# kocurvik/mdrp

Measured on NVIDIA B200. Metric: image_pairs_per_sec, higher is better.
Workload: dtype f64

## Files before the change

mdrp_b200/csrc/repose_b200.cu:

```cuda
#include <cuda.h>
#include <cuda_runtime.h>
#include <algorithm>
#include <cstdio>
#include <cstdlib>
#include <cstring>
#include <string>
#include <type_traits>
#include <vector>

#include "rp_kernels.cuh"

using namespace rp;

namespace {

std::string g_create_error;

struct DevBuf {
    void *p = nullptr;
    size_t cap = 0;
    cudaError_t reserve(size_t bytes) {
        if (bytes <= cap) return cudaSuccess;
        if (p) cudaFree(p);
        p = nullptr;
        cap = 0;
        const size_t want = bytes + bytes / 8 + 256;
        cudaError_t e = cudaMalloc(&p, want);
        if (e == cudaSuccess) cap = want;
        return e;
    }
    void release() {
        if (p) cudaFree(p);
        p = nullptr;
        cap = 0;
    }
    template <class T>
    T *as() const { return (T *)p; }
};

enum { B_OFFS, B_PAIRS, B_PTS64, B_PTS32, B_BEAR, B_SAMPLES, B_MODELS, B_HYPITER, B_SCORE, B_COUNT, B_SEGCNT,
       B_ITEMPFX, B_SCALARS, B_EVENTS, B_NEVENTS, B_LOMODELS, B_LOOFEV, B_LOCOUNT, B_PROBLIST, B_LOSCORE,
       B_LOCNT, B_LOITEMPFX, B_BEST, B_FINSTART, B_FINSCORE, B_FINCNT, B_ONES, B_ONEPFX, B_ENABLE, B_STATS,
       B_PTS32P, B_UB, B_LB, B_FIRSTCNT, B_FIRSTPFX, B_B0, B_S0, B_SURVLIST, B_SURVCNT, B_SURVPFX, B_WAVECUR, B_WAVECNT,
       B_MASK, B_IN_X1, B_IN_X2, B_IN_D1, B_IN_D2, B_IN_CAMS, B_TMP0, B_TMP1, B_TMP2,
       B_MASK_B, B_IN_X1_B, B_IN_X2_B, B_IN_D1_B, B_IN_D2_B, B_IN_CAMS_B, B_TMP0_B, B_TMP1_B,
       B_FEAT, B_TCOUT, B_TCLIST, B_TCLISTCNT, B_TCLISTPFX, B_PAIRCNT, B_TCPFX, B_TCSPLIT,
       B_PAIRFLAGS, B_SUB_IDX, B_SUB_SRC, B_SUB_DST, B_SUB_X1, B_SUB_X2, B_SUB_D1, B_SUB_D2, B_SUB_CAMS, B_SUB_MODELS,
       B_SUB_STATS, B_SUB_MASK,
       B_STG_X1, B_STG_X2, B_STG_D1, B_STG_D2, B_STG_X1_B, B_STG_X2_B, B_STG_D1_B, B_STG_D2_B,
       B_QUAL, B_QUAL_B, B_ORDOFFS, B_ORDOFFS_B, B_PERM, B_PERM_B, B_KSORT, B_KSORT_B, B_ORDSCR,
       B_GATHER_Q,
       B_RF_INIT, B_RF_INIT_B, B_RF_SUB, B_RF_SUB_B, B_RF_NINL, B_RF_NINL_B, B_NBUF };

struct Scalars {
    int n_items, n_lo_items, n_one_items, n_prob, n_pairs_scalar, any_flag, reserved0, n_first_items;
    int n_surv_items, bound_work, lm_work, score_work;
    unsigned long long point_scores, lm_iters, n_survivors, evaluated_ps;
    long long n_hyp;
    int n_tc_items, n_tcsel_items;
    unsigned long long tc_evaluated, tc_selected, lm_flops;
};

constexpr int N_EVENTS = 29;

}

struct rp_ctx {
    int device = 0;
    int sms = 148;
    std::string err;
    int64_t launches = 0;
    cudaStream_t stream = nullptr;
    cudaStream_t copy_stream = nullptr;
    DevBuf buf[B_NBUF];
    cudaEvent_t ev[N_EVENTS];
    double last_ms[16] = {0};
    double prev_h2d_ms = 0.0, prev_dev_ms = 0.0;
    int64_t last_cnt[16] = {0};
    size_t workspace_budget = (size_t)80 << 30;
    bool prune = true;
    int head = HB;
    bool waves = true;
    int lm_warp = 0xf;
    int head_small = 32;
    int mid_end = 256;
    int mid_ends[4] = {256, 0, 0, 0}, n_mid = 1;
    bool tc = true;
    int tc_two_pass = -115;
    void *encode_tiled = nullptr;
    int ev_cap0 = EV;
    std::vector<int32_t> pair_status;
    int occ_score[4] = {0}, occ_lm[4] = {0};
};

namespace {

#define CK(call)                                                                                     \
    do {                                                                                             \
        cudaError_t e_ = (call);                                                                     \
        if (e_ != cudaSuccess) {                                                                     \
            char b_[512];                                                                            \
            snprintf(b_, sizeof b_, "%s failed at %s:%d: %s", #call, __FILE__, __LINE__,             \
                     cudaGetErrorString(e_));                                                        \
            ctx->err = b_;                                                                           \
            return RP_ERR_CUDA;                                                                      \
        }                                                                                            \
    } while (0)

#define LAUNCHED()                                                                                   \
    do {                                                                                             \
        ctx->launches++;                                                                             \
        CK(cudaGetLastError());                                                                      \
    } while (0)

inline int cdiv(long long a, long long b) { return (int)((a + b - 1) / b); }

// ... 25 lines not shown
}

template <class K>
int occupancy_grid(rp_ctx *ctx, K kernel, int threads) {
    int nb = 0;
    if (cudaOccupancyMaxActiveBlocksPerMultiprocessor(&nb, kernel, threads, 0) != cudaSuccess || nb < 1) nb = 1;
    return nb * ctx->sms;
}

int launch_score(rp_ctx *ctx, bool pose, bool mask, const ScoreArgs &args, cudaStream_t st) {
    int grid;
    ScoreArgs a = args;
    a.work_counter = &ctx->buf[B_SCALARS].as<Scalars>()->score_work;
    CK(cudaMemsetAsync(a.work_counter, 0, sizeof(int), st));
    if (pose) {
        if (mask) { grid = occupancy_grid(ctx, score_kernel<true, true>, SCORE_THREADS); score_kernel<true, true><<<grid, SCORE_THREADS, 0, st>>>(a); }
        else { grid = occupancy_grid(ctx, score_kernel<true, false>, SCORE_THREADS); score_kernel<true, false><<<grid, SCORE_THREADS, 0, st>>>(a); }
    } else {
        if (mask) { grid = occupancy_grid(ctx, score_kernel<false, true>, SCORE_THREADS); score_kernel<false, true><<<grid, SCORE_THREADS, 0, st>>>(a); }
        else { grid = occupancy_grid(ctx, score_kernel<false, false>, SCORE_THREADS); score_kernel<false, false><<<grid, SCORE_THREADS, 0, st>>>(a); }
    }
    LAUNCHED();
    return RP_OK;
}

int launch_bound(rp_ctx *ctx, bool pose, const BoundArgs &a, cudaStream_t st) {
    CK(cudaMemsetAsync(a.work_counter, 0, sizeof(int), st));
    if (pose) bound_kernel<true><<<occupancy_grid(ctx, bound_kernel<true>, SCORE_THREADS), SCORE_THREADS, 0, st>>>(a);
    else bound_kernel<false><<<occupancy_grid(ctx, bound_kernel<false>, SCORE_THREADS), SCORE_THREADS, 0, st>>>(a);
    LAUNCHED();
    return RP_OK;
}

int launch_lm(rp_ctx *ctx, int variant, const LMArgs &a, long long expected_problems, cudaStream_t st) {
    ctx->launches++;
    (void)expected_problems;
    LMArgs la = a;
    la.work_counter = &ctx->buf[B_SCALARS].as<Scalars>()->lm_work;
    la.warp_kernel = (ctx->lm_warp >> variant) & 1;
    la.warp_single = (ctx->lm_warp >> 4) & 1;
    CK(cudaMemsetAsync(la.work_counter, 0, sizeof(int), st));
    CK((cudaError_t)launch_lm_kernel(ctx->sms, variant, la, st));
    return RP_OK;
}

int launch_solve(rp_ctx *ctx, int variant, const SolveArgs &a, int n_pairs, cudaStream_t st) {
    dim3 grid(a.nseg, n_pairs);
    const bool generic = getenv("RP_SOLVE_GENERIC") != nullptr;
    switch (variant) {
    case RP_CALIB:
        if (generic) solve_kernel<RP_CALIB><<<grid, SOLVE_THREADS, 0, st>>>(a);
        else solve2_kernel<P3PCand><<<grid, SOLVE_THREADS, 0, st>>>(a);
        break;
    case RP_CALIB_SHIFT:
        if (generic) solve_kernel<RP_CALIB_SHIFT><<<grid, SOLVE_THREADS, 0, st>>>(a);
        else solve2_kernel<ShiftCand><<<grid, SOLVE_THREADS, 0, st>>>(a);
        break;
    case RP_SHARED:
        if (generic) solve_kernel<RP_SHARED><<<grid, SOLVE_THREADS, 0, st>>>(a);
        else solve2_kernel<FocalCand><<<grid, SOLVE_THREADS, 0, st>>>(a);
        break;
    default: solve_kernel<RP_VARYING><<<grid, SOLVE_THREADS, 0, st>>>(a); break;
    }
    LAUNCHED();
    return RP_OK;
}

__global__ void valid_ones_kernel(int n_pairs, const PairParams *pairs, int *ones) {
    const int i = blockIdx.x * blockDim.x + threadIdx.x;
    if (i < n_pairs) ones[i] = pairs[i].valid ? 1 : 0;
}

__global__ void stage_points_kernel(int n, const double *x1, const double *x2, double sq_thr, Pt64 *pts64,
// ... 294 lines not shown
            }
        }
        CK(cudaEventRecord(ev[20], st));
        rc = cascade(from, 0, ctx->tc_two_pass, use_tc ? ev[22] : nullptr, ev[21]);
        if (rc) return rc;
    }
    CK(cudaEventRecord(ev[4], st));
    {
        ScanArgs a;
        a.n_pairs = P; a.nseg = nseg; a.seg_count = seg_count; a.score = score; a.count = count;
        a.events = B[B_EVENTS].as<int>(); a.n_events = B[B_NEVENTS].as<int>(); a.ev_cap = ev_cap;
        a.pair_flags = B[B_PAIRFLAGS].as<int>(); a.any_flag = &sc->any_flag;
        scan_kernel<<<cdiv((long long)P * 32, 256), 256, 0, st>>>(a);
        LAUNCHED();
        LoPrepArgs l;
        l.n_pairs = P; l.nseg = nseg; l.events = a.events; l.n_events = a.n_events; l.hyp_iter = hyp_iter; l.ev_cap = ev_cap;
        l.models = models; l.lo_models = B[B_LOMODELS].as<Model>(); l.lo_of_event = B[B_LOOFEV].as<int>();
        l.lo_count = B[B_LOCOUNT].as<int>(); l.prob_list = B[B_PROBLIST].as<int>(); l.n_prob = &sc->n_prob;
        lo_prepare_kernel<<<cdiv(P, 128), 128, 0, st>>>(l);
        LAUNCHED();
    }
    CK(cudaEventRecord(ev[5], st));
    LMArgs la;
    memset(&la, 0, sizeof la);
    la.pairs = pairs; la.pts64 = pts64; la.d1 = io.d1; la.d2 = io.d2;
    la.weight_sampson = opt.weight_sampson; la.gradient_tol = 1e-10; la.step_tol = 1e-8;
    la.initial_lambda = 1e-3; la.min_lambda = 1e-10; la.max_lambda = 1e10;
    la.loss_scale_override = -1.0; la.scale_reproj_override = -1.0;
    la.lm_iters = &sc->lm_iters;
    la.lm_flops = &sc->lm_flops;
    {
        la.prob_list = B[B_PROBLIST].as<int>(); la.n_prob = &sc->n_prob; la.prob_per_pair = ev_cap;
        la.models = B[B_LOMODELS].as<Model>(); la.use_final = 0;
        int rc = launch_lm(ctx, variant, la, (long long)P * 8, st);
        if (rc) return rc;
    }
    CK(cudaEventRecord(ev[6], st));
    {
        build_items_kernel<<<1, 1024, 0, st>>>(P, B[B_LOCOUNT].as<int>(), B[B_LOITEMPFX].as<int>(), &sc->n_lo_items, nullptr);
        LAUNCHED();
        ScoreArgs s2 = sa;
        s2.slot_list = nullptr; s2.list_stride = 0;
        s2.n_groups = P; s2.grp_stride = ev_cap; s2.grp_per_pair = 1; s2.grp_cnt = B[B_LOCOUNT].as<int>();
        s2.item_prefix = B[B_LOITEMPFX].as<int>(); s2.n_items = &sc->n_lo_items; s2.models = B[B_LOMODELS].as<Model>();
        s2.score = B[B_LOSCORE].as<double>(); s2.count = B[B_LOCNT].as<int>(); s2.point_scores = nullptr;
        int rc = launch_score(ctx, pose, false, s2, st);
        if (rc) return rc;
        MergeArgs m;
        m.n_pairs = P; m.nseg = nseg; m.iters = iters; m.pairs = pairs; m.events = B[B_EVENTS].as<int>();
        m.min_iterations = opt.min_iterations; m.max_iterations = opt.max_iterations;
        m.dyn_num_trials_mult = opt.dyn_num_trials_mult; m.log_prob_missing = log(1.0 - opt.success_prob);
        m.hyp_iter = hyp_iter; m.ev_cap = ev_cap; m.pair_flags = B[B_PAIRFLAGS].as<int>(); m.any_flag = &sc->any_flag;
        m.n_events = B[B_NEVENTS].as<int>(); m.lo_of_event = B[B_LOOFEV].as<int>(); m.score = score; m.count = count;
        m.models = models; m.lo_score = B[B_LOSCORE].as<double>(); m.lo_count_inl = B[B_LOCNT].as<int>();
        m.lo_models = B[B_LOMODELS].as<Model>(); m.lo_count = B[B_LOCOUNT].as<int>();
        m.best = B[B_BEST].as<Model>(); m.stats = B[B_STATS].as<rp_stats>(); m.final_start = B[B_FINSTART].as<Model>();
        merge_kernel<<<cdiv(P, 128), 128, 0, st>>>(m);
        LAUNCHED();
        la.prob_list = nullptr; la.n_prob = &sc->n_pairs_scalar; la.prob_per_pair = 1;
        la.models = B[B_FINSTART].as<Model>(); la.use_final = 0;
        rc = launch_lm(ctx, variant, la, P, st);
        if (rc) return rc;
        valid_ones_kernel<<<cdiv(P, 256), 256, 0, st>>>(P, pairs, B[B_ONES].as<int>());
        LAUNCHED();
        build_items_kernel<<<1, 1024, 0, st>>>(P, B[B_ONES].as<int>(), B[B_ONEPFX].as<int>(), &sc->n_one_items, nullptr);
        LAUNCHED();
        ScoreArgs s3 = s2;
        s3.grp_stride = 1; s3.grp_cnt = B[B_ONES].as<int>(); s3.item_prefix = B[B_ONEPFX].as<int>();
        s3.n_items = &sc->n_one_items; s3.models = B[B_FINSTART].as<Model>();
        s3.score = B[B_FINSCORE].as<double>(); s3.count = B[B_FINCNT].as<int>();
        rc = launch_score(ctx, pose, false, s3, st);
        if (rc) return rc;
        Merge2Args m2;
        m2.n_pairs = P; m2.pairs = pairs; m2.refined = B[B_FINSTART].as<Model>(); m2.ref_score = B[B_FINSCORE].as<double>();
        m2.ref_count = B[B_FINCNT].as<int>(); m2.best = B[B_BEST].as<Model>(); m2.stats = B[B_STATS].as<rp_stats>();
        merge2_kernel<<<cdiv(P, 128), 128, 0, st>>>(m2);
        LAUNCHED();
        CK(cudaMemsetAsync(io.masks_out, 0, (size_t)std::max<long long>(N, 1), st));
        ScoreArgs s4 = s3;
        s4.models = B[B_BEST].as<Model>(); s4.mask = io.masks_out;
        rc = launch_score(ctx, pose, true, s4, st);
        if (rc) return rc;
    }
    CK(cudaEventRecord(ev[7], st));
    {
        enable_final_kernel<<<cdiv(P, 256), 256, 0, st>>>(P, B[B_STATS].as<rp_stats>(), B[B_ENABLE].as<int>());
        LAUNCHED();
        la.prob_list = nullptr; la.n_prob = &sc->n_pairs_scalar; la.prob_per_pair = 1;
        la.models = B[B_BEST].as<Model>(); la.use_final = 1; la.mask = io.masks_out; la.enable = B[B_ENABLE].as<int>();
        la.max_iterations = (int)opt.bundle_max_iterations; la.loss_type = opt.loss_type;
        la.gradient_tol = opt.gradient_tol; la.step_tol = opt.step_tol; la.initial_lambda = opt.initial_lambda;
        la.min_lambda = opt.min_lambda; la.max_lambda = opt.max_lambda;
        int rc = launch_lm(ctx, variant, la, P, st);
        if (rc) return rc;
        finalize_kernel<<<cdiv(P, 256), 256, 0, st>>>(P, variant, pairs, B[B_BEST].as<Model>());
        LAUNCHED();
        CK(cudaMemcpyAsync(io.models_out, B[B_BEST].p, sizeof(Model) * P, cudaMemcpyDeviceToDevice, st));
        CK(cudaMemcpyAsync(io.stats_out, B[B_STATS].p, sizeof(rp_stats) * P, cudaMemcpyDeviceToDevice, st));
    }
    CK(cudaEventRecord(ev[8], st));
    CK(cudaMemcpyAsync(&h_sc, sc, sizeof h_sc, cudaMemcpyDeviceToHost, st));
    CK(cudaStreamSynchronize(st));
    for (int i = 0; i < 8; ++i) {
        float ms = 0.f;
        CK(cudaEventElapsedTime(&ms, ev[i], ev[i + 1]));
        ctx->last_ms[i] += ms;
    }
    {
        float ms = 0.f;
        CK(cudaEventElapsedTime(&ms, ev[0], ev[8]));
        ctx->last_ms[8] += ms;
    }
    ctx->last_cnt[0] += h_sc.n_hyp;
    ctx->last_cnt[1] += (int64_t)h_sc.point_scores;
    ctx->last_cnt[2] += h_sc.n_prob + P;
    ctx->last_cnt[3] += (int64_t)h_sc.lm_iters;
    ctx->last_cnt[4] += 1;
    ctx->last_cnt[6] += (int64_t)h_sc.evaluated_ps;
    if (ctx->prune) {
        float msb = 0.f;
        CK(cudaEventElapsedTime(&msb, use_tc ? ev[22] : ev[20], ev[21]));
        ctx->last_ms[11] += msb;
        if (use_tc) {
            CK(cudaEventElapsedTime(&msb, ev[20], ev[22]));
            ctx->last_ms[12] += msb;
        }
    }
    ctx->last_cnt[8] += (int64_t)h_sc.tc_evaluated;
    ctx->last_cnt[9] += (int64_t)h_sc.tc_selected;
    ctx->last_cnt[10] += (int64_t)h_sc.lm_flops;
    ctx->last_cnt[5] += ctx->prune ? (int64_t)h_sc.n_survivors + std::min<int64_t>(h_sc.n_hyp, (int64_t)P * ((ctx->tc && ctx->mid_end > ctx->head_small) ? ctx->head_small : ctx->head)) : h_sc.n_hyp;
    ctx->last_cnt[7] = ctx->head;
    flags.assign((size_t)P, 0);
    if (h_sc.any_flag) {
        CK(cudaMemcpyAsync(flags.data(), B[B_PAIRFLAGS].p, sizeof(int) * (size_t)P, cudaMemcpyDeviceToHost, st));
        CK(cudaStreamSynchronize(st));
    }
    return RP_OK;
}

size_t bytes_per_pair(int iters, long long avg_points, int ev_cap = EV, size_t input_bytes = 0) {
    const int nseg = std::max(1, cdiv(iters, SEG));
    const size_t slots_pp = (size_t)nseg * 4 * SEG;
    return slots_pp * (sizeof(Model) + 4 + 8 + 4 + 12 + 8) + (size_t)iters * 12 + (size_t)ev_cap * (sizeof(Model) + 24) +
           (size_t)avg_points * (sizeof(Pt64) + 32 + sizeof(Bear) + 1 + 128 + input_bytes) + 1024;
}

template <class In>
int launch_widen(rp_ctx *ctx, long long n, const In *x1, const In *x2, const In *d1, const In *d2, double *wx1,
                 double *wx2, double *wd1, double *wd2, cudaStream_t st, const int *perm = nullptr,
                 const long long *offsets = nullptr, long long base = 0, int n_pairs = 0) {
    if (n <= 0) return RP_OK;
    const int grid = std::min<long long>(cdiv(perm ? n : 2 * n, 256), 16LL * ctx->sms);
    widen_inputs_kernel<In><<<grid, 256, 0, st>>>(n, x1, x2, d1, d2, perm, offsets, base, n_pairs, wx1, wx2, wd1, wd2);
    LAUNCHED();
    return RP_OK;
}

int launch_order(rp_ctx *ctx, int P, long long n, const int64_t *h_offsets, const long long *d_offsets, long long base,
                 const float *quality, int *perm, cudaStream_t st) {
    if (n <= 0) return RP_OK;
    long long max_n = 0;
    for (int p = 0; p < P; ++p) max_n = std::max<long long>(max_n, h_offsets[p + 1] - h_offsets[p]);
    OrderArgs a;
    a.offsets = d_offsets; a.base = base; a.quality = quality; a.perm = perm;
    a.smem_cap = (int)std::min<long long>(max_n, ORDER_SMEM_CAP);
    a.gkeys = nullptr; a.gidx = nullptr;
    if (max_n > ORDER_SMEM_CAP) {
        CK(ctx->buf[B_ORDSCR].reserve(12 * (size_t)n));
        a.gkeys = ctx->buf[B_ORDSCR].as<unsigned>();
        a.gidx = (int *)(a.gkeys + 2 * n);
    }
    order_by_quality_kernel<<<P, ORDER_THREADS, (size_t)ORDER_SMEM_PER_POINT * a.smem_cap, st>>>(a);
    LAUNCHED();
    return RP_OK;
}

int launch_scatter_masks(rp_ctx *ctx, int P, long long n, const long long *d_offsets, long long base, const int *perm,
// ... 379 lines not shown
    PairParams *pairs = B[B_PAIRS].as<PairParams>();
    Model *work = B[B_BEST].as<Model>();
    int *enable = B[B_ENABLE].as<int>();
    Scalars h_sc;
    memset(&h_sc, 0, sizeof h_sc);
    h_sc.n_pairs_scalar = P;
    CK(cudaMemcpyAsync(sc, &h_sc, sizeof h_sc, cudaMemcpyHostToDevice, st));
    CK(cudaMemcpyAsync(B[B_OFFS].p, io.h_offsets_rel, sizeof(long long) * (P + 1), cudaMemcpyHostToDevice, st));
    {
        PrepareArgs a;
        a.variant = variant; a.n_pairs = P; a.offsets = B[B_OFFS].as<long long>();
        a.x1 = io.x1; a.x2 = io.x2; a.cams = io.cams;
        a.max_epipolar_error = opt.max_epipolar_error; a.max_reproj_error = opt.max_reproj_error;
        a.loss_scale = opt.loss_scale;
        a.pts64 = B[B_PTS64].as<Pt64>(); a.pts32 = B[B_PTS32].as<float4>(); a.bear = B[B_BEAR].as<Bear>();
        a.pairs = pairs; a.pts32p = B[B_PTS32P].as<float>();
        prepare_kernel<<<cdiv((long long)P * 32, 256), 256, 0, st>>>(a);
        LAUNCHED();
    }
    refine_import_kernel<<<cdiv((long long)P * 32, 256), 256, 0, st>>>(P, variant, pairs, io.subset, io.init, work, enable,
                                                                      io.bstats_out);
    LAUNCHED();
    {
        LMArgs la;
        memset(&la, 0, sizeof la);
        la.pairs = pairs; la.pts64 = B[B_PTS64].as<Pt64>(); la.d1 = io.d1; la.d2 = io.d2;
        la.weight_sampson = opt.weight_sampson;
        la.loss_scale_override = -1.0; la.scale_reproj_override = -1.0;
        la.prob_list = nullptr; la.n_prob = &sc->n_pairs_scalar; la.prob_per_pair = 1;
        la.models = work; la.use_final = 1; la.mask = io.subset; la.enable = enable; la.stats = io.bstats_out;
        la.max_iterations = (int)opt.bundle_max_iterations; la.loss_type = opt.loss_type;
        la.gradient_tol = opt.gradient_tol; la.step_tol = opt.step_tol; la.initial_lambda = opt.initial_lambda;
        la.min_lambda = opt.min_lambda; la.max_lambda = opt.max_lambda;
        int rc = launch_lm(ctx, variant, la, P, st);
        if (rc) return rc;
    }
    if (io.inliers_out) {
        valid_ones_kernel<<<cdiv(P, 256), 256, 0, st>>>(P, pairs, B[B_ONES].as<int>());
        LAUNCHED();
        build_items_kernel<<<1, 1024, 0, st>>>(P, B[B_ONES].as<int>(), B[B_ONEPFX].as<int>(), &sc->n_one_items, nullptr);
        LAUNCHED();
        if (N > 0) CK(cudaMemsetAsync(io.inliers_out, 0, (size_t)N, st));
        ScoreArgs s;
        memset(&s, 0, sizeof s);
        s.n_groups = P; s.grp_stride = 1; s.grp_per_pair = 1; s.grp_cnt = B[B_ONES].as<int>();
        s.item_prefix = B[B_ONEPFX].as<int>(); s.n_items = &sc->n_one_items; s.pairs = pairs; s.models = work;
        s.pts32 = B[B_PTS32].as<float4>(); s.pts64 = B[B_PTS64].as<Pt64>(); s.bear = B[B_BEAR].as<Bear>();
        s.score = B[B_FINSCORE].as<double>(); s.count = B[B_FINCNT].as<int>(); s.mask = io.inliers_out;
        int rc = launch_score(ctx, pose, true, s, st);
        if (rc) return rc;
    }
    refine_export_kernel<<<cdiv(P, 256), 256, 0, st>>>(P, variant, pairs, enable, io.init, work, B[B_FINCNT].as<int>(),
                                                       io.models_out, io.num_inliers_out);
    LAUNCHED();
    return RP_OK;
}

size_t refine_bytes_per_pair(long long avg_points, bool host_io, bool f32) {
    const size_t io_pt = 48 + 1 + 1 + (host_io && f32 ? 24 : 0);
    const size_t io_pair = 2 * sizeof(Model) + sizeof(rp_bundle_stats) + 64 + 8;
    const size_t sets = host_io ? 2 : 1;
    return (size_t)avg_points * (32 + 16 + 16 + 48 + sets * io_pt) + sizeof(PairParams) + sizeof(Model) + 32 +
           sets * io_pair + 64;
}

template <class In>
int refine_impl(rp_ctx *ctx, int variant, int64_t n_pairs, const int64_t *offsets, const In *x1, const In *x2,
                const In *d1, const In *d2, const double *cams, const rp_options *opt_in, const rp_model *init,
                const uint8_t *subset, rp_model *models, rp_bundle_stats *bstats, int64_t *num_inliers, uint8_t *inliers,
                bool host_io, cudaStream_t st) {
    constexpr bool f32 = std::is_same<In, float>::value;
    if (!ctx) return RP_ERR_INVALID;
    if (n_pairs > 0 && (!x1 || !x2 || !d1 || !d2)) return fail(ctx, RP_ERR_INVALID, "null data pointer");
    if (n_pairs > 0 && (!init || !models)) return fail(ctx, RP_ERR_INVALID, "null init / models");
    int rc = check_common(ctx, variant, n_pairs, offsets, opt_in);
    if (rc) return rc;
    CK(cudaSetDevice(ctx->device));
    rp_options opt = *opt_in;
    if (variant == RP_CALIB && opt.estimate_shift) variant = RP_CALIB_SHIFT;
    const bool pose = variant == RP_CALIB || variant == RP_CALIB_SHIFT;
    if (pose && !cams && n_pairs > 0) return fail(ctx, RP_ERR_INVALID, "calibrated variants need cams");
    if (n_pairs == 0) return RP_OK;
    const bool score = num_inliers || inliers;
    const long long Ntot = offsets[n_pairs] - offsets[0];
    int64_t chunk = (int64_t)std::max<size_t>(1, ctx->workspace_budget / refine_bytes_per_pair(Ntot / n_pairs + 1, host_io, f32));
    chunk = std::min<int64_t>(chunk, 32768);
    if (host_io && n_pairs >= 1024) chunk = std::min<int64_t>(chunk, (n_pairs + 3) / 4);
    const int64_t n_chunks = (n_pairs + chunk - 1) / chunk;
    std::vector<int64_t> bounds((size_t)n_chunks + 1);
    for (int64_t i = 0; i <= n_chunks; ++i) bounds[(size_t)i] = (n_pairs * i) / n_chunks;
    DevBuf *B = ctx->buf;
    static const int IN_X1[2] = {B_IN_X1, B_IN_X1_B}, IN_X2[2] = {B_IN_X2, B_IN_X2_B}, IN_D1[2] = {B_IN_D1, B_IN_D1_B},
                     IN_D2[2] = {B_IN_D2, B_IN_D2_B}, IN_CAMS[2] = {B_IN_CAMS, B_IN_CAMS_B}, STG_X1[2] = {B_STG_X1, B_STG_X1_B},
                     STG_X2[2] = {B_STG_X2, B_STG_X2_B}, STG_D1[2] = {B_STG_D1, B_STG_D1_B}, STG_D2[2] = {B_STG_D2, B_STG_D2_B},
                     INIT[2] = {B_RF_INIT, B_RF_INIT_B}, SUB[2] = {B_RF_SUB, B_RF_SUB_B}, OUT_M[2] = {B_TMP0, B_TMP0_B},
                     OUT_S[2] = {B_TMP1, B_TMP1_B}, OUT_K[2] = {B_MASK, B_MASK_B}, OUT_N[2] = {B_RF_NINL, B_RF_NINL_B};
// ... 104 lines not shown

extern "C" {

int rp_create(int device, rp_ctx **out) {
    if (!out) return RP_ERR_INVALID;
    *out = nullptr;
    int ndev = 0;
    cudaError_t e = cudaGetDeviceCount(&ndev);
    if (e != cudaSuccess || ndev == 0) {
        g_create_error = std::string("no CUDA device: ") + cudaGetErrorString(e);
        return RP_ERR_NO_DEVICE;
    }
    if (device < 0 || device >= ndev) {
        g_create_error = "device index out of range";
        return RP_ERR_INVALID;
    }
    cudaDeviceProp prop;
    if (cudaGetDeviceProperties(&prop, device) != cudaSuccess || prop.major < 10) {
        g_create_error = "device is not sm_100-class (this library only ships sm_100a code)";
        return RP_ERR_NO_DEVICE;
    }
    rp_ctx *ctx = new rp_ctx();
    ctx->device = device;
    ctx->sms = prop.multiProcessorCount;
    if (cudaSetDevice(device) != cudaSuccess || cudaStreamCreateWithFlags(&ctx->stream, cudaStreamNonBlocking) != cudaSuccess ||
        cudaStreamCreateWithFlags(&ctx->copy_stream, cudaStreamNonBlocking) != cudaSuccess) {
        g_create_error = "cudaSetDevice / stream creation failed";
        delete ctx;
        return RP_ERR_CUDA;
    }
    for (auto &ev : ctx->ev) cudaEventCreate(&ev);
    if (const char *np = getenv("RP_NO_PRUNE")) ctx->prune = !(np[0] == '1');
    if (const char *nw = getenv("RP_NO_WAVES")) ctx->waves = !(nw[0] == '1');
    if (const char *lw = getenv("RP_LM_WARP")) ctx->lm_warp = atoi(lw) & 0x1f;
    if (const char *hs = getenv("RP_HEAD_SMALL")) { const int v = atoi(hs); if (v >= 0 && v <= 256 && v % 32 == 0) ctx->head_small = v; }
    if (const char *me = getenv("RP_MID_END")) {
        int n = 0, vals[4] = {0, 0, 0, 0};
        bool ok = true;
        for (const char *p = me; *p && n < 4;) {
            const int v = atoi(p);
            if (v < 0 || v > SEG || v % 32 != 0 || (n && v <= vals[n - 1])) ok = false;
            vals[n++] = v;
            while (*p && *p != ',') ++p;
            if (*p == ',') ++p;
        }
        if (ok && n) { ctx->n_mid = n; for (int k = 0; k < 4; ++k) ctx->mid_ends[k] = vals[k]; ctx->mid_end = vals[n - 1]; }
    }
    if (const char *nt = getenv("RP_NO_TC")) ctx->tc = !(nt[0] == '1');
    if (const char *sp = getenv("RP_TC_SPLIT")) { const int v = atoi(sp); if (v >= 1 && v <= 15) ctx->tc_two_pass = v; }
    if (const char *ap = getenv("RP_TC_ADAPT_PCT")) { const int v = atoi(ap); if (v >= 50 && v <= 200) ctx->tc_two_pass = -v; }
    if (const char *op = getenv("RP_TC_ONE_PASS")) { if (op[0] == '1') ctx->tc_two_pass = 0; }
    if (const char *ec = getenv("RP_EV_CAP")) { const int v = atoi(ec); if (v >= 1 && v <= EV) ctx->ev_cap0 = v; }
    {
        cudaDriverEntryPointQueryResult qres;
        void *fn = nullptr;
        if (cudaGetDriverEntryPoint("cuTensorMapEncodeTiled", &fn, cudaEnableDefault, &qres) != cudaSuccess || !fn ||
            qres != cudaDriverEntryPointSuccess ||
            cudaFuncSetAttribute(tc::tc_count_kernel<0>, cudaFuncAttributeMaxDynamicSharedMemorySize, tc::SMEM_BYTES) != cudaSuccess ||
            cudaFuncSetAttribute(order_by_quality_kernel, cudaFuncAttributeMaxDynamicSharedMemorySize,
                                 ORDER_SMEM_PER_POINT * ORDER_SMEM_CAP) != cudaSuccess) {
            g_create_error = "tensor-map entry point / shared-memory opt-in unavailable (driver too old for sm_100a TMA?)";
            rp_destroy(ctx);
            return RP_ERR_CUDA;
        }
        ctx->encode_tiled = fn;
    }
    if (const char *hd = getenv("RP_HEAD")) { const int v = atoi(hd); if (v == 32 || v == 64 || v == 96 || v == 128) ctx->head = v; }
// ... 356 lines not shown
        (n_models > 0 && !models) || (n_points > 0 && (!x1 || !x2 || !d1 || !d2)))
        return fail(ctx, RP_ERR_INVALID, "bad argument");
    if (n_models == 0) return RP_OK;
    CK(cudaSetDevice(ctx->device));
    cudaStream_t st = ctx->stream;
    DevBuf *B = ctx->buf;
    int rc = stage_pair(ctx, n_points, x1, x2, 1.0, st);
    if (rc) return rc;
    const size_t nn = (size_t)std::max<int64_t>(n_points, 1);
    CK(B[B_IN_D1].reserve(8 * nn)); CK(B[B_IN_D2].reserve(8 * nn)); CK(B[B_MASK].reserve(nn));
    CK(B[B_MODELS].reserve(sizeof(Model) * (size_t)n_models)); CK(B[B_SCALARS].reserve(sizeof(Scalars)));
    CK(B[B_TMP2].reserve(sizeof(rp_bundle_stats) * (size_t)n_models));
    CK(cudaMemcpyAsync(B[B_IN_D1].p, d1, 8 * (size_t)n_points, cudaMemcpyHostToDevice, st));
    CK(cudaMemcpyAsync(B[B_IN_D2].p, d2, 8 * (size_t)n_points, cudaMemcpyHostToDevice, st));
    if (mask) CK(cudaMemcpyAsync(B[B_MASK].p, mask, (size_t)n_points, cudaMemcpyHostToDevice, st));
    CK(cudaMemcpyAsync(B[B_MODELS].p, models, sizeof(Model) * (size_t)n_models, cudaMemcpyHostToDevice, st));
    Scalars h;
    memset(&h, 0, sizeof h);
    h.n_prob = (int)n_models;
    Scalars *sc = B[B_SCALARS].as<Scalars>();
    CK(cudaMemcpyAsync(sc, &h, sizeof h, cudaMemcpyHostToDevice, st));
    LMArgs la;
    memset(&la, 0, sizeof la);
    la.prob_list = nullptr; la.n_prob = &sc->n_prob; la.prob_per_pair = 1 << 30;
    la.pairs = B[B_PAIRS].as<PairParams>(); la.pts64 = B[B_PTS64].as<Pt64>();
    la.d1 = B[B_IN_D1].as<double>(); la.d2 = B[B_IN_D2].as<double>();
    la.mask = mask ? B[B_MASK].as<unsigned char>() : nullptr; la.enable = nullptr;
    la.models = B[B_MODELS].as<Model>(); la.use_final = 1;
    la.max_iterations = (int)opt->max_iterations; la.loss_type = opt->loss_type;
    la.weight_sampson = weight_sampson; la.gradient_tol = opt->gradient_tol; la.step_tol = opt->step_tol;
    la.initial_lambda = opt->initial_lambda; la.min_lambda = opt->min_lambda; la.max_lambda = opt->max_lambda;
    la.loss_scale_override = opt->loss_scale; la.scale_reproj_override = scale_reproj;
    la.stats = B[B_TMP2].as<rp_bundle_stats>(); la.lm_iters = nullptr;
    rc = launch_lm(ctx, variant, la, n_models, st);
    if (rc) return rc;
    CK(cudaMemcpyAsync(models, B[B_MODELS].p, sizeof(Model) * (size_t)n_models, cudaMemcpyDeviceToHost, st));
    if (stats) CK(cudaMemcpyAsync(stats, B[B_TMP2].p, sizeof(rp_bundle_stats) * (size_t)n_models, cudaMemcpyDeviceToHost, st));
    CK(cudaStreamSynchronize(st));
    return RP_OK;
}

}

namespace {

template <class T>
int gather_depths_impl(rp_ctx *ctx, const float *depth1, int h1, int w1, const float *depth2, int h2, int w2,
                       const float *kp1, const float *kp2, const float *quality, int64_t n, T *x1, T *x2, T *d1, T *d2,
                       float *quality_out, int64_t *n_out, void *stream, bool with_q) {
    if (!ctx || n < 0 || !n_out || h1 <= 0 || w1 <= 0 || h2 <= 0 || w2 <= 0 ||
        (n > 0 && (!depth1 || !depth2 || !kp1 || !kp2 || !x1 || !x2 || !d1 || !d2)))
        return fail(ctx, RP_ERR_INVALID, "bad argument");
    if (with_q && n > 0 && (!quality || !quality_out)) return fail(ctx, RP_ERR_INVALID, "null quality / quality_out");
    *n_out = 0;
    if (n == 0) return RP_OK;
    CK(cudaSetDevice(ctx->device));
    cudaStream_t st = stream ? (cudaStream_t)stream : ctx->stream;
    CK(ctx->buf[B_SCALARS].reserve(sizeof(Scalars)));
    long long *d_n = (long long *)ctx->buf[B_SCALARS].p;
    gather_depths_kernel<T><<<1, 1024, 0, st>>>(depth1, h1, w1, depth2, h2, w2, kp1, kp2, quality, (long long)n,
                                                x1, x2, d1, d2, quality_out, d_n);
    LAUNCHED();
    long long h_n = 0;
    CK(cudaMemcpyAsync(&h_n, d_n, sizeof h_n, cudaMemcpyDeviceToHost, st));
    CK(cudaStreamSynchronize(st));
    *n_out = h_n;
    return RP_OK;
// ... 148 lines not shown
```

mdrp_b200/csrc/repose_lm.cu:

```cuda
#include "rp_lm_kernel.cuh"

#ifndef RP_LM_THREADS
#define RP_LM_THREADS 128
#endif

namespace rp {

template <class K>
static int occupancy_grid(int sms, K kernel, int threads) {
    int nb = 0;
    if (cudaOccupancyMaxActiveBlocksPerMultiprocessor(&nb, kernel, threads, 0) != cudaSuccess || nb < 1) nb = 1;
    return nb * sms;
}

template <int VARIANT, int NP>
static void launch_variant(int sms, const LMArgs &a, cudaStream_t st) {
    if (a.warp_kernel && (a.prob_list || a.warp_single) && !a.mask && !a.use_final)
        lm_warp_kernel<VARIANT, NP, RP_LOSS_TRUNCATED>
            <<<occupancy_grid(sms, lm_warp_kernel<VARIANT, NP, RP_LOSS_TRUNCATED>, LMW_WPB[VARIANT] * 32), LMW_WPB[VARIANT] * 32, 0, st>>>(a);
    else if (!a.use_final)
        lm_kernel<VARIANT, NP, RP_LM_THREADS, RP_LOSS_TRUNCATED>
            <<<occupancy_grid(sms, lm_kernel<VARIANT, NP, RP_LM_THREADS, RP_LOSS_TRUNCATED>, RP_LM_THREADS), RP_LM_THREADS, 0, st>>>(a);
    else if (a.loss_type == RP_LOSS_TRUNCATED_CAUCHY)
        lm_kernel<VARIANT, NP, RP_LM_THREADS, RP_LOSS_TRUNCATED_CAUCHY>
            <<<occupancy_grid(sms, lm_kernel<VARIANT, NP, RP_LM_THREADS, RP_LOSS_TRUNCATED_CAUCHY>, RP_LM_THREADS), RP_LM_THREADS, 0, st>>>(a);
    else if (a.loss_type == RP_LOSS_CAUCHY)
        lm_kernel<VARIANT, NP, RP_LM_THREADS, RP_LOSS_CAUCHY>
            <<<occupancy_grid(sms, lm_kernel<VARIANT, NP, RP_LM_THREADS, RP_LOSS_CAUCHY>, RP_LM_THREADS), RP_LM_THREADS, 0, st>>>(a);
    else
        lm_kernel<VARIANT, NP, RP_LM_THREADS, -1>
            <<<occupancy_grid(sms, lm_kernel<VARIANT, NP, RP_LM_THREADS, -1>, RP_LM_THREADS), RP_LM_THREADS, 0, st>>>(a);
}

int launch_lm_kernel(int sms, int variant, const LMArgs &a, cudaStream_t st) {
    switch (variant) {
    case RP_CALIB: launch_variant<RP_CALIB, 7>(sms, a, st); break;
    case RP_CALIB_SHIFT: launch_variant<RP_CALIB_SHIFT, 9>(sms, a, st); break;
    case RP_SHARED: launch_variant<RP_SHARED, 8>(sms, a, st); break;
    default: launch_variant<RP_VARYING, 9>(sms, a, st); break;
    }
    return (int)cudaGetLastError();
}

}
```

mdrp_b200/csrc/rp_kernels.cuh:

```cuda
#pragma once
#include <cuda_runtime.h>
#include "rp_types.cuh"
#include "rp_solvers.cuh"
#include "rp_score.cuh"
#include "rp_lm_kernel.cuh"
#include "rp_tc.cuh"
#include "rp_order.cuh"

namespace rp {

struct PrepareArgs {
    int variant;
    int n_pairs;
    const long long *offsets;
    const double *x1, *x2;
    const double *cams;
    double max_epipolar_error, max_reproj_error, loss_scale;
    Pt64 *pts64;
    float4 *pts32;
    float *pts32p;
    Bear *bear;
    PairParams *pairs;
};

// ... 1333 lines not shown
    const int *ref_count;
    Model *best;
    rp_stats *stats;
};
__global__ void merge2_kernel(Merge2Args a) {
    const int pair = blockIdx.x * blockDim.x + threadIdx.x;
    if (pair >= a.n_pairs) return;
    const PairParams pp = a.pairs[pair];
    if (!pp.valid) return;
    rp_stats st = a.stats[pair];
    st.refinements++;
    const double rs = a.ref_score[pair];
    if (rs < st.model_score) {
        st.num_inliers = a.ref_count[pair];
        a.best[pair] = a.refined[pair];
    }
    st.inlier_ratio = (double)st.num_inliers / (double)pp.n;
    a.stats[pair] = st;
}

__global__ void enable_final_kernel(int n_pairs, const rp_stats *stats, int *enable) {
    const int pair = blockIdx.x * blockDim.x + threadIdx.x;
    if (pair < n_pairs) enable[pair] = stats[pair].num_inliers > 3;
}
__global__ void finalize_kernel(int n_pairs, int variant, const PairParams *pairs, Model *best) {
    const int pair = blockIdx.x * blockDim.x + threadIdx.x;
    if (pair >= n_pairs) return;
    if (variant == RP_SHARED || variant == RP_VARYING) {
        best[pair].f1 *= pairs[pair].nscale;
        best[pair].f2 *= pairs[pair].nscale;
    }
}

__global__ void refine_import_kernel(int n_pairs, int variant, const PairParams *pairs, const unsigned char *subset,
                                     const Model *init, Model *work, int *enable, rp_bundle_stats *bstats) {
    const int pair = (blockIdx.x * blockDim.x + threadIdx.x) >> 5;
    const int lane = threadIdx.x & 31;
    if (pair >= n_pairs) return;
    const PairParams pp = pairs[pair];
    int cnt = pp.n;
    if (subset) {
        cnt = 0;
        const unsigned char *s = subset + pp.off;
        for (int b0 = 0; b0 < pp.n; b0 += 32) cnt += __popc(__ballot_sync(0xffffffffu, b0 + lane < pp.n && s[b0 + lane]));
    }
    if (lane != 0) return;
    Model m = init[pair];
    if (variant == RP_SHARED || variant == RP_VARYING) {
        m.f1 /= pp.nscale;
        m.f2 /= pp.nscale;
    }
    work[pair] = m;
    enable[pair] = cnt > 3;
    if (bstats) bstats[pair] = rp_bundle_stats{};
}

__global__ void refine_export_kernel(int n_pairs, int variant, const PairParams *pairs, const int *enable,
                                     const Model *init, const Model *work, const int *count, Model *out,
                                     long long *num_inliers) {
    const int pair = blockIdx.x * blockDim.x + threadIdx.x;
    if (pair >= n_pairs) return;
    const PairParams pp = pairs[pair];
    Model m;
    if (enable[pair]) {
        m = work[pair];
        if (variant == RP_SHARED || variant == RP_VARYING) {
// ... 223 lines not shown
```

mdrp_b200/csrc/rp_lm_kernel.cuh:

```cuda
#pragma once
#include "rp_types.cuh"
#include "rp_lm.cuh"
#include <type_traits>

#ifndef RP_LM_UNROLL
#define RP_LM_UNROLL 1
#endif
#ifndef RP_LM_MIN_BLOCKS
#define RP_LM_MIN_BLOCKS 3
#endif

namespace rp {

constexpr int LM_UNROLL = RP_LM_UNROLL;

struct LMArgs {
    const int *prob_list;
    const int *n_prob;
    int prob_per_pair;
    const PairParams *pairs;
    const Pt64 *pts64;
    const double *d1, *d2;
    const unsigned char *mask;
    const int *enable;
    Model *models;
    int use_final;
    int max_iterations, loss_type;
    double weight_sampson, gradient_tol, step_tol, initial_lambda, min_lambda, max_lambda;
    double loss_scale_override;
    double scale_reproj_override;
    rp_bundle_stats *stats;
    unsigned long long *lm_iters;
    unsigned long long *lm_flops;
    int *work_counter;
    int warp_kernel;
    int warp_single;
};

constexpr int LM_LIST_CAP = 16384;

template <int MAXV, int CNT, int O>
struct ReduceScatter {
    static RP_D void run(double (&v)[MAXV], int lane, int &base, int &lim) {
        constexpr int H = (CNT + 1) / 2;
        const bool up = (lane & O) != 0;
#pragma unroll
        for (int i = 0; i < H; ++i) {
            const double lo = v[i];
            const double hi = (i + H < CNT) ? v[i + H] : 0.0;
            const double send = up ? lo : hi, keep = up ? hi : lo;
            v[i] = keep + __shfl_xor_sync(0xffffffffu, send, O);
        }
        if (up) { base += H; lim = max(lim - H, 0); }
        else lim = min(lim, H);
        ReduceScatter<MAXV, H, O / 2>::run(v, lane, base, lim);
    }
};
template <int MAXV, int CNT>
struct ReduceScatter<MAXV, CNT, 0> {
    static RP_D void run(double (&)[MAXV], int, int &, int &) {}
};
template <int CNT, int STEPS>
struct ReduceScatterLeft {
    static constexpr int value = ReduceScatterLeft<(CNT + 1) / 2, STEPS - 1>::value;
};
template <int CNT>
struct ReduceScatterLeft<CNT, 0> {
    static constexpr int value = CNT;
};
// ... 191 lines not shown
        }
        __syncthreads();
        if (tid == 0) {
            a.models[prob] = cur;
            if (a.stats) {
                rp_bundle_stats s;
                s.iterations = it; s.initial_cost = initial_cost; s.cost = cost; s.lambda = lambda;
                s.invalid_steps = invalid_steps; s.step_norm = step_norm; s.grad_norm = grad_norm;
                a.stats[prob] = s;
            }
            if (a.lm_iters) atomicAdd(a.lm_iters, (unsigned long long)it);
        }
        if (a.lm_flops) {
#pragma unroll
            for (int o = 16; o > 0; o >>= 1) rows += __shfl_xor_sync(0xffffffffu, rows, o);
            if (lane == 0) {
                const unsigned long long fl = (rows & 0x1fffffull) * LM_FLOPS[VARIANT][1] + ((rows >> 21) & 0x1fffffull) * LM_FLOPS[VARIANT][2] +
                                              ((rows >> 42) & 0x1fffffull) * LM_FLOPS[VARIANT][3] +
                                              (wid == 0 ? (unsigned long long)passes * m_work * LM_FLOPS[VARIANT][0] : 0ull);
                atomicAdd(a.lm_flops, fl);
            }
        }
    }
}

#ifndef RP_LMW_WPB
#define RP_LMW_WPB 4, 4, 4, 4
#endif
#ifndef RP_LMW_BPS
#define RP_LMW_BPS 3, 2, 2, 2
#endif
constexpr int LMW_WPB[4] = {RP_LMW_WPB};
constexpr int LMW_BPS[4] = {RP_LMW_BPS};
constexpr int LMW_MAX_WPB = 8;
constexpr int LMW_SLOTS = 3;

RP_D void cp_async16(void *dst_smem, const void *src) {
    asm volatile("cp.async.cg.shared.global [%0], [%1], 16;" ::"r"((unsigned)__cvta_generic_to_shared(dst_smem)), "l"(src) : "memory");
}
RP_D void cp_async8(void *dst_smem, const void *src) {
    asm volatile("cp.async.ca.shared.global [%0], [%1], 8;" ::"r"((unsigned)__cvta_generic_to_shared(dst_smem)), "l"(src) : "memory");
}
RP_D void cp_async_commit() { asm volatile("cp.async.commit_group;" ::: "memory"); }
template <int N>
RP_D void cp_async_wait() { asm volatile("cp.async.wait_group %0;" ::"n"(N) : "memory"); }

template <int VARIANT, int NP, int LOSS>
__global__ void __launch_bounds__(LMW_WPB[VARIANT] * 32, LMW_BPS[VARIANT]) lm_warp_kernel(LMArgs a) {
    constexpr int NA = NP * (NP + 1) / 2;
    struct __align__(16) Slot { double x[4]; double d1, d2; };
    struct WarpState {
        Model cur, trial;
        double sA[NA], sg[NP];
        double step_norm;
        int stop;
    };
    __shared__ WarpState ws_all[LMW_WPB[VARIANT]];
    __shared__ Slot ring_all[LMW_WPB[VARIANT]][LMW_SLOTS][32];
    const int lane = threadIdx.x & 31, wid = threadIdx.x >> 5;
    WarpState &W = ws_all[wid];
    Slot (*ring)[32] = ring_all[wid];
    const int n_prob = *a.n_prob;
    for (;;) {
        int pj = 0;
        if (lane == 0) pj = atomicAdd(a.work_counter, 1);
        pj = __shfl_sync(0xffffffffu, pj, 0);
        if (pj >= n_prob) break;
        const int prob = a.prob_list ? a.prob_list[pj] : pj;
        const int pair = prob / a.prob_per_pair;
        const PairParams pp = a.pairs[pair];
        if (!pp.valid) continue;
        if (a.enable && !a.enable[pair]) continue;
        LMParams P;
        P.weight_sampson = a.weight_sampson;
        P.scale_reproj = a.scale_reproj_override >= 0.0 ? a.scale_reproj_override : pp.scale_reproj;
        if (a.use_final) {
            P.loss_type = LOSS >= 0 ? LOSS : a.loss_type;
            P.loss_scale = a.loss_scale_override > 0.0 ? a.loss_scale_override : pp.final_loss_scale;
        } else {
            P.loss_type = RP_LOSS_TRUNCATED;
            P.loss_scale = pp.lo_loss_scale;
        }
        P.inv_t2 = 1.0 / (P.loss_scale * P.loss_scale);
        const int max_it = a.use_final ? a.max_iterations : 25;
        const int n = pp.n;
        const Pt64 *pts = a.pts64 + pp.off;
        const double *d1 = a.d1 + pp.off, *d2 = a.d2 + pp.off;
        __syncwarp();
        if (lane == 0) { W.cur = a.models[prob]; W.stop = 0; }
        __syncwarp();

        auto fetch = [&](int i, int s) {
            if (i < n) {
                Slot *d = &ring[s][lane];
                const char *src = reinterpret_cast<const char *>(pts + i);
                cp_async16(&d->x[0], src);
                cp_async16(&d->x[2], src + 16);
                cp_async8(&d->d1, d1 + i);
                cp_async8(&d->d2, d2 + i);
            }
            cp_async_commit();
        };

        unsigned long long rows = 0;
        auto warp_pass = [&](const Model &m, NormalEq<NP> &N, auto jac_tag) -> double {
            constexpr bool jac = decltype(jac_tag)::value;
            const LMFrame F = make_frame(m);
            double c = 0.0;
            LogProd lp;
            lp.init();
            if (jac) N.clear();
            fetch(lane, 0);
            fetch(lane + 32, 1);
            int s = 0;
            for (int i = lane; i < n; i += 32) {
                cp_async_wait<1>();
                const Slot q = ring[s][lane];
                int s2 = s + 2; if (s2 >= LMW_SLOTS) s2 -= LMW_SLOTS;
                fetch(i + 64, s2);
                if (jac) c += point_eval<VARIANT, NP, LOSS>(F, P, q.x[0], q.x[1], q.x[2], q.x[3], q.d1, q.d2, N, rows, lp);
                else c += point_cost<VARIANT, LOSS>(F, P, q.x[0], q.x[1], q.x[2], q.x[3], q.d1, q.d2, lp);
                if (++s == LMW_SLOTS) s = 0;
            }
            cp_async_wait<0>();
            if (lm_loss_may_be_cauchy(LOSS)) c += P.loss_scale * P.loss_scale * lp.total(P.weight_sampson);
            return warp_sum(c);
        };
        auto reduce_normal = [&](NormalEq<NP> &N) {
            constexpr int NV = NA + NP, LEFT = ReduceScatterLeft<NV, 5>::value;
            double v[NV];
#pragma unroll
            for (int i = 0; i < NA; ++i) v[i] = N.A[i];
// ... 89 lines not shown
```

Before: 79910.

## Route final Cauchy LM refinement through warp kernel with compacted inlier points

Adds a compaction kernel that packs the masked inlier points and depths of each pair into a contiguous array of 48-byte slots and records per-pair counts. The final LM refinement for Cauchy and truncated-Cauchy losses now runs on the warp-per-problem kernel, which reads these compacted slots, instead of on the block kernel. This avoids iterating over masked-out points and allows one 16-byte async copy for the depths. The default lm_warp bitmask turns the path on for two variants. The cost is an extra kernel launch and workspace for the compacted copy.

```diff
diff --git a/mdrp_b200/csrc/repose_b200.cu b/mdrp_b200/csrc/repose_b200.cu
--- a/mdrp_b200/csrc/repose_b200.cu
+++ b/mdrp_b200/csrc/repose_b200.cu
@@ -50,7 +50,8 @@
        B_STG_X1, B_STG_X2, B_STG_D1, B_STG_D2, B_STG_X1_B, B_STG_X2_B, B_STG_D1_B, B_STG_D2_B,
        B_QUAL, B_QUAL_B, B_ORDOFFS, B_ORDOFFS_B, B_PERM, B_PERM_B, B_KSORT, B_KSORT_B, B_ORDSCR,
        B_GATHER_Q,
-       B_RF_INIT, B_RF_INIT_B, B_RF_SUB, B_RF_SUB_B, B_RF_NINL, B_RF_NINL_B, B_NBUF };
+       B_RF_INIT, B_RF_INIT_B, B_RF_SUB, B_RF_SUB_B, B_RF_NINL, B_RF_NINL_B,
+       B_LMCPTS, B_LMCCNT, B_NBUF };
 
 struct Scalars {
     int n_items, n_lo_items, n_one_items, n_prob, n_pairs_scalar, any_flag, reserved0, n_first_items;
@@ -81,7 +82,7 @@
     bool prune = true;
     int head = HB;
     bool waves = true;
-    int lm_warp = 0xf;
+    int lm_warp = 0xa0f;
     int head_small = 32;
     int mid_end = 256;
     int mid_ends[4] = {256, 0, 0, 0}, n_mid = 1;
@@ -173,13 +174,22 @@
     return RP_OK;
 }
 
-int launch_lm(rp_ctx *ctx, int variant, const LMArgs &a, long long expected_problems, cudaStream_t st) {
+int launch_lm(rp_ctx *ctx, int variant, const LMArgs &a, int n_pairs, long long n_points, cudaStream_t st) {
     ctx->launches++;
-    (void)expected_problems;
     LMArgs la = a;
     la.work_counter = &ctx->buf[B_SCALARS].as<Scalars>()->lm_work;
     la.warp_kernel = (ctx->lm_warp >> variant) & 1;
-    la.warp_single = (ctx->lm_warp >> 4) & 1;
+    la.warp_single = (ctx->lm_warp >> (4 + variant)) & 1;
+    if (a.use_final && ((ctx->lm_warp >> (8 + variant)) & 1) &&(a.loss_type == RP_LOSS_TRUNCATED_CAUCHY || a.loss_type == RP_LOSS_CAUCHY)) {
+        DevBuf *B = ctx->buf;
+        CK(B[B_LMCPTS].reserve(sizeof(LMSlot) * (size_t)std::max<long long>(n_points, 1)));
+        CK(B[B_LMCCNT].reserve(sizeof(int) * (size_t)std::max(n_pairs, 1)));
+        la.cpts = B[B_LMCPTS].as<LMSlot>();
+        la.ccount = B[B_LMCCNT].as<int>();
+        lm_compact_kernel<<<cdiv(n_pairs, COMPACT_WARPS), COMPACT_WARPS * 32, 0, st>>>(n_pairs, a.pairs, a.mask, a.enable, a.pts64, a.d1,
+                                                                                   a.d2, B[B_LMCPTS].as<LMSlot>(), B[B_LMCCNT].as<int>());
+        LAUNCHED();
+    }
     CK(cudaMemsetAsync(la.work_counter, 0, sizeof(int), st));
     CK((cudaError_t)launch_lm_kernel(ctx->sms, variant, la, st));
     return RP_OK;
@@ -540,7 +550,7 @@
     {
         la.prob_list = B[B_PROBLIST].as<int>(); la.n_prob = &sc->n_prob; la.prob_per_pair = ev_cap;
         la.models = B[B_LOMODELS].as<Model>(); la.use_final = 0;
-        int rc = launch_lm(ctx, variant, la, (long long)P * 8, st);
+        int rc = launch_lm(ctx, variant, la, P, N, st);
         if (rc) return rc;
     }
     CK(cudaEventRecord(ev[6], st));
@@ -567,7 +577,7 @@
         LAUNCHED();
         la.prob_list = nullptr; la.n_prob = &sc->n_pairs_scalar; la.prob_per_pair = 1;
         la.models = B[B_FINSTART].as<Model>(); la.use_final = 0;
-        rc = launch_lm(ctx, variant, la, P, st);
+        rc = launch_lm(ctx, variant, la, P, N, st);
         if (rc) return rc;
         valid_ones_kernel<<<cdiv(P, 256), 256, 0, st>>>(P, pairs, B[B_ONES].as<int>());
         LAUNCHED();
@@ -599,7 +609,7 @@
         la.max_iterations = (int)opt.bundle_max_iterations; la.loss_type = opt.loss_type;
         la.gradient_tol = opt.gradient_tol; la.step_tol = opt.step_tol; la.initial_lambda = opt.initial_lambda;
         la.min_lambda = opt.min_lambda; la.max_lambda = opt.max_lambda;
-        int rc = launch_lm(ctx, variant, la, P, st);
+        int rc = launch_lm(ctx, variant, la, P, N, st);
         if (rc) return rc;
         finalize_kernel<<<cdiv(P, 256), 256, 0, st>>>(P, variant, pairs, B[B_BEST].as<Model>());
         LAUNCHED();
@@ -651,7 +661,7 @@
     const int nseg = std::max(1, cdiv(iters, SEG));
     const size_t slots_pp = (size_t)nseg * 4 * SEG;
     return slots_pp * (sizeof(Model) + 4 + 8 + 4 + 12 + 8) + (size_t)iters * 12 + (size_t)ev_cap * (sizeof(Model) + 24) +
-           (size_t)avg_points * (sizeof(Pt64) + 32 + sizeof(Bear) + 1 + 128 + input_bytes) + 1024;
+           (size_t)avg_points * (sizeof(Pt64) + 32 + sizeof(Bear) + 1 + 128 + sizeof(LMSlot) + input_bytes) + 1024;
 }
 
 template <class In>
@@ -1097,7 +1107,7 @@
         la.max_iterations = (int)opt.bundle_max_iterations; la.loss_type = opt.loss_type;
         la.gradient_tol = opt.gradient_tol; la.step_tol = opt.step_tol; la.initial_lambda = opt.initial_lambda;
         la.min_lambda = opt.min_lambda; la.max_lambda = opt.max_lambda;
-        int rc = launch_lm(ctx, variant, la, P, st);
+        int rc = launch_lm(ctx, variant, la, P, N, st);
         if (rc) return rc;
     }
     if (io.inliers_out) {
@@ -1125,8 +1135,8 @@
     const size_t io_pt = 48 + 1 + 1 + (host_io && f32 ? 24 : 0);
     const size_t io_pair = 2 * sizeof(Model) + sizeof(rp_bundle_stats) + 64 + 8;
     const size_t sets = host_io ? 2 : 1;
-    return (size_t)avg_points * (32 + 16 + 16 + 48 + sets * io_pt) + sizeof(PairParams) + sizeof(Model) + 32 +
-           sets * io_pair + 64;
+    return (size_t)avg_points * (32 + 16 + 16 + 48 + sizeof(LMSlot) + sets * io_pt) + sizeof(PairParams) + sizeof(Model) +
+           36 + sets * io_pair + 64;
 }
 
 template <class In>
@@ -1297,7 +1307,7 @@
     for (auto &ev : ctx->ev) cudaEventCreate(&ev);
     if (const char *np = getenv("RP_NO_PRUNE")) ctx->prune = !(np[0] == '1');
     if (const char *nw = getenv("RP_NO_WAVES")) ctx->waves = !(nw[0] == '1');
-    if (const char *lw = getenv("RP_LM_WARP")) ctx->lm_warp = atoi(lw) & 0x1f;
+    if (const char *lw = getenv("RP_LM_WARP")) ctx->lm_warp = atoi(lw) & 0xfff;
     if (const char *hs = getenv("RP_HEAD_SMALL")) { const int v = atoi(hs); if (v >= 0 && v <= 256 && v % 32 == 0) ctx->head_small = v; }
     if (const char *me = getenv("RP_MID_END")) {
         int n = 0, vals[4] = {0, 0, 0, 0};
@@ -1720,7 +1730,7 @@
     la.initial_lambda = opt->initial_lambda; la.min_lambda = opt->min_lambda; la.max_lambda = opt->max_lambda;
     la.loss_scale_override = opt->loss_scale; la.scale_reproj_override = scale_reproj;
     la.stats = B[B_TMP2].as<rp_bundle_stats>(); la.lm_iters = nullptr;
-    rc = launch_lm(ctx, variant, la, n_models, st);
+    rc = launch_lm(ctx, variant, la, 1, n_points, st);
     if (rc) return rc;
     CK(cudaMemcpyAsync(models, B[B_MODELS].p, sizeof(Model) * (size_t)n_models, cudaMemcpyDeviceToHost, st));
     if (stats) CK(cudaMemcpyAsync(stats, B[B_TMP2].p, sizeof(rp_bundle_stats) * (size_t)n_models, cudaMemcpyDeviceToHost, st));
diff --git a/mdrp_b200/csrc/repose_lm.cu b/mdrp_b200/csrc/repose_lm.cu
--- a/mdrp_b200/csrc/repose_lm.cu
+++ b/mdrp_b200/csrc/repose_lm.cu
@@ -13,11 +13,20 @@
     return nb * sms;
 }
 
+template <int VARIANT, int NP, int LOSS>
+static void launch_warp(int sms, const LMArgs &a, cudaStream_t st) {
+    constexpr int threads = lmw_wpb(VARIANT, LOSS) * 32;
+    lm_warp_kernel<VARIANT, NP, LOSS><<<occupancy_grid(sms, lm_warp_kernel<VARIANT, NP, LOSS>, threads), threads, 0, st>>>(a);
+}
+
 template <int VARIANT, int NP>
 static void launch_variant(int sms, const LMArgs &a, cudaStream_t st) {
     if (a.warp_kernel && (a.prob_list || a.warp_single) && !a.mask && !a.use_final)
-        lm_warp_kernel<VARIANT, NP, RP_LOSS_TRUNCATED>
-            <<<occupancy_grid(sms, lm_warp_kernel<VARIANT, NP, RP_LOSS_TRUNCATED>, LMW_WPB[VARIANT] * 32), LMW_WPB[VARIANT] * 32, 0, st>>>(a);
+        launch_warp<VARIANT, NP, RP_LOSS_TRUNCATED>(sms, a, st);
+    else if (a.use_final && a.cpts && a.loss_type == RP_LOSS_TRUNCATED_CAUCHY)
+        launch_warp<VARIANT, NP, RP_LOSS_TRUNCATED_CAUCHY>(sms, a, st);
+    else if (a.use_final && a.cpts && a.loss_type == RP_LOSS_CAUCHY)
+        launch_warp<VARIANT, NP, RP_LOSS_CAUCHY>(sms, a, st);
     else if (!a.use_final)
         lm_kernel<VARIANT, NP, RP_LM_THREADS, RP_LOSS_TRUNCATED>
             <<<occupancy_grid(sms, lm_kernel<VARIANT, NP, RP_LM_THREADS, RP_LOSS_TRUNCATED>, RP_LM_THREADS), RP_LM_THREADS, 0, st>>>(a);
diff --git a/mdrp_b200/csrc/rp_kernels.cuh b/mdrp_b200/csrc/rp_kernels.cuh
--- a/mdrp_b200/csrc/rp_kernels.cuh
+++ b/mdrp_b200/csrc/rp_kernels.cuh
@@ -1389,6 +1389,34 @@
     }
 }
 
+constexpr int COMPACT_WARPS = 8;
+__global__ void __launch_bounds__(COMPACT_WARPS * 32)
+    lm_compact_kernel(int n_pairs, const PairParams *__restrict__ pairs, const unsigned char *__restrict__ mask,
+                      const int *__restrict__ enable, const Pt64 *__restrict__ pts64, const double *__restrict__ d1,
+                      const double *__restrict__ d2, LMSlot *__restrict__ out, int *__restrict__ count) {
+    const int lane = threadIdx.x & 31;
+    const int pair = blockIdx.x * COMPACT_WARPS + (threadIdx.x >> 5);
+    if (pair >= n_pairs) return;
+    const PairParams pp = pairs[pair];
+    if (!pp.valid || (enable && !enable[pair])) return;
+    const long long off = pp.off;
+    int pos = 0;
+    for (int b0 = 0; b0 < pp.n; b0 += 32) {
+        const int k = b0 + lane;
+        const bool in = k < pp.n && (!mask || mask[off + k]);
+        const unsigned bal = __ballot_sync(0xffffffffu, in);
+        if (in) {
+            const Pt64 p = pts64[off + k];
+            LMSlot s;
+            s.x[0] = p.x1_0; s.x[1] = p.x1_1; s.x[2] = p.x2_0; s.x[3] = p.x2_1;
+            s.d1 = d1[off + k]; s.d2 = d2[off + k];
+            out[off + pos + __popc(bal & ((1u << lane) - 1u))] = s;
+        }
+        pos += __popc(bal);
+    }
+    if (lane == 0) count[pair] = pos;
+}
+
 __global__ void refine_import_kernel(int n_pairs, int variant, const PairParams *pairs, const unsigned char *subset,
                                      const Model *init, Model *work, int *enable, rp_bundle_stats *bstats) {
     const int pair = (blockIdx.x * blockDim.x + threadIdx.x) >> 5;
diff --git a/mdrp_b200/csrc/rp_lm_kernel.cuh b/mdrp_b200/csrc/rp_lm_kernel.cuh
--- a/mdrp_b200/csrc/rp_lm_kernel.cuh
+++ b/mdrp_b200/csrc/rp_lm_kernel.cuh
@@ -13,6 +13,8 @@
 namespace rp {
 
 constexpr int LM_UNROLL = RP_LM_UNROLL;
+
+struct __align__(16) LMSlot { double x[4]; double d1, d2; };
 
 struct LMArgs {
     const int *prob_list;
@@ -35,6 +37,8 @@
     int *work_counter;
     int warp_kernel;
     int warp_single;
+    const LMSlot *cpts;
+    const int *ccount;
 };
 
 constexpr int LM_LIST_CAP = 16384;
@@ -292,6 +296,16 @@
 #endif
 constexpr int LMW_WPB[4] = {RP_LMW_WPB};
 constexpr int LMW_BPS[4] = {RP_LMW_BPS};
+#ifndef RP_LMWF_WPB
+#define RP_LMWF_WPB 4, 4, 4, 4
+#endif
+#ifndef RP_LMWF_BPS
+#define RP_LMWF_BPS 2, 2, 2, 2
+#endif
+constexpr int LMWF_WPB[4] = {RP_LMWF_WPB};
+constexpr int LMWF_BPS[4] = {RP_LMWF_BPS};
+RP_HD constexpr int lmw_wpb(int variant, int loss) { return loss == RP_LOSS_TRUNCATED ? LMW_WPB[variant] : LMWF_WPB[variant]; }
+RP_HD constexpr int lmw_bps(int variant, int loss) { return loss == RP_LOSS_TRUNCATED ? LMW_BPS[variant] : LMWF_BPS[variant]; }
 constexpr int LMW_MAX_WPB = 8;
 constexpr int LMW_SLOTS = 3;
 
@@ -306,17 +320,19 @@
 RP_D void cp_async_wait() { asm volatile("cp.async.wait_group %0;" ::"n"(N) : "memory"); }
 
 template <int VARIANT, int NP, int LOSS>
-__global__ void __launch_bounds__(LMW_WPB[VARIANT] * 32, LMW_BPS[VARIANT]) lm_warp_kernel(LMArgs a) {
+__global__ void __launch_bounds__(lmw_wpb(VARIANT, LOSS) * 32, lmw_bps(VARIANT, LOSS)) lm_warp_kernel(LMArgs a) {
     constexpr int NA = NP * (NP + 1) / 2;
-    struct __align__(16) Slot { double x[4]; double d1, d2; };
+    constexpr int WPB = lmw_wpb(VARIANT, LOSS);
+    constexpr bool compact = LOSS != RP_LOSS_TRUNCATED;
+    using Slot = LMSlot;
     struct WarpState {
         Model cur, trial;
         double sA[NA], sg[NP];
         double step_norm;
         int stop;
     };
-    __shared__ WarpState ws_all[LMW_WPB[VARIANT]];
-    __shared__ Slot ring_all[LMW_WPB[VARIANT]][LMW_SLOTS][32];
+    __shared__ WarpState ws_all[WPB];
+    __shared__ Slot ring_all[WPB][LMW_SLOTS][32];
     const int lane = threadIdx.x & 31, wid = threadIdx.x >> 5;
     WarpState &W = ws_all[wid];
     Slot (*ring)[32] = ring_all[wid];
@@ -343,7 +359,8 @@
         }
         P.inv_t2 = 1.0 / (P.loss_scale * P.loss_scale);
         const int max_it = a.use_final ? a.max_iterations : 25;
-        const int n = pp.n;
+        const int n = compact ? a.ccount[pair] : pp.n;
+        const Slot *cpts = compact ? a.cpts + pp.off : nullptr;
         const Pt64 *pts = a.pts64 + pp.off;
         const double *d1 = a.d1 + pp.off, *d2 = a.d2 + pp.off;
         __syncwarp();
@@ -353,11 +370,18 @@
         auto fetch = [&](int i, int s) {
             if (i < n) {
                 Slot *d = &ring[s][lane];
-                const char *src = reinterpret_cast<const char *>(pts + i);
-                cp_async16(&d->x[0], src);
-                cp_async16(&d->x[2], src + 16);
-                cp_async8(&d->d1, d1 + i);
-                cp_async8(&d->d2, d2 + i);
+                if constexpr (compact) {
+                    const char *src = reinterpret_cast<const char *>(cpts + i);
+                    cp_async16(&d->x[0], src);
+                    cp_async16(&d->x[2], src + 16);
+                    cp_async16(&d->d1, src + 32);
+                } else {
+                    const char *src = reinterpret_cast<const char *>(pts + i);
+                    cp_async16(&d->x[0], src);
+                    cp_async16(&d->x[2], src + 16);
+                    cp_async8(&d->d1, d1 + i);
+                    cp_async8(&d->d2, d2 + i);
+                }
             }
             cp_async_commit();
         };
```

Result: no change. 80200 (median of 6 runs) (+0.4%).
